# hwwang55/GraphGAN

Measured on NVIDIA H100. Metric: sampled negative edges/sec (D-sampling pass), higher is better.
Workload: dtype f32

## Files before the change

### graphgan_b200/_cabi.py

```python
import ctypes as C
import os

from . import _build

_LIB = None
ABI_VERSION = 11


class GGError(RuntimeError):
    pass


class WalkDesc(C.Structure):
    _fields_ = [
        ("n_node", C.c_int64), ("ld", C.c_int32),
        ("emb", C.c_void_p), ("bias", C.c_void_p), ("indptr", C.c_void_p), ("adj", C.c_void_p),
        ("n_roots", C.c_int64), ("roots", C.c_void_p), ("tree_bits", C.c_void_p), ("tree_words", C.c_int64),
        ("walk_ptr", C.c_void_p),
        ("n_walks", C.c_int64), ("for_d", C.c_int32), ("rng_mode", C.c_int32), ("d1_bits", C.c_void_p),
        ("seed", C.c_uint64), ("pass_tag", C.c_uint32), ("max_path", C.c_int32),
        ("stream", C.c_void_p), ("n_stream", C.c_int64), ("update_ratio", C.c_double),
        ("max_cand", C.c_int32), ("phase_mask", C.c_int32),
        ("samples", C.c_void_p), ("status", C.c_void_p), ("first_edge", C.c_void_p), ("wsteps", C.c_void_p),
        ("wsuml", C.c_void_p), ("paths", C.c_void_p), ("path_len", C.c_void_p), ("counters", C.c_void_p),
        ("scratch", C.c_void_p), ("scratch_bytes", C.c_int64), ("work_counter", C.c_void_p),
        ("edge_score", C.c_void_p), ("root_q", C.c_void_p), ("rq_ptr", C.c_void_p),
        ("hub_threshold", C.c_int32), ("no_tma", C.c_int32), ("walk_slot", C.c_void_p),
        ("s1_nq", C.c_int64), ("s1_slot", C.c_void_p), ("s1_ptr", C.c_void_p), ("s1_cnt", C.c_void_p), ("s1_n", C.c_void_p),
        ("s1_q", C.c_void_p), ("s1_ids", C.c_void_p), ("first_idx", C.c_void_p), ("s1_order", C.c_void_p), ("walk_order", C.c_void_p),
        ("flat_buf", C.c_void_p), ("flat_bytes", C.c_int64), ("flat_steps", C.c_int32), ("flat_reserved", C.c_int32),
    ]


_P, _I32, _I64, _F = C.c_void_p, C.c_int32, C.c_int64, C.c_float
SIGNATURES = {
    "gg_last_error": (C.c_char_p, []),
    "gg_abi_version": (C.c_int, []),
    "gg_hub_scores": (C.c_int, [_I64, _P, _P, _P, _P, _I32, _P, _P]),
    "gg_root_cdf": (C.c_int, [C.POINTER(WalkDesc), _P, _P, _P]),
    "gg_walk_scratch_bytes": (C.c_int, [_I32, C.POINTER(_I64)]),
    "gg_walk_flat_bytes": (C.c_int, [_I64, _I32, _I32, C.POINTER(_I64)]),
    "gg_walk_sample": (C.c_int, [C.POINTER(WalkDesc), _P]),
    "gg_generator_dist_scratch_bytes": (C.c_int, [_I64, _I64, _I64, C.POINTER(_I64)]),
    "gg_generator_dist": (C.c_int, [C.POINTER(WalkDesc), _P, _P, _P, _I64, _P]),
    "gg_game_value_scratch_bytes": (C.c_int, [_I64, _I64, C.POINTER(_I64)]),
    "gg_game_value": (C.c_int, [_I64, _I32, _P, _P, _P, _P, _I64, _P, _P, _P, _P, _P, _P, _P, _I64, _P]),
    "gg_game_value_grad_scratch_bytes": (C.c_int, [_I64, _I64, _I64, C.POINTER(_I64)]),
    "gg_game_value_grad": (C.c_int, [C.POINTER(WalkDesc), _P, _P, _P, _P, _P, _P, _P, _P, _P, _P, _I64, _P]),
    "gg_game_value_grad_d_scratch_bytes": (C.c_int, [_I64, _I32, _I64, C.POINTER(_I64)]),
    "gg_game_value_grad_d": (C.c_int, [_I64, _I32, _P, _P, _P, _P, _I64, _P, _P, _P, _P, _P, _P, _I64, _P]),
    "gg_expected_g_grad_scratch_bytes": (C.c_int, [_I64, _I64, _I64, _I32, C.POINTER(_I64)]),
    "gg_expected_g_grad": (C.c_int, [C.POINTER(WalkDesc), _P, _P, _I32, _P, _P, _P, _P, _P, _I64, _P]),
    "gg_walk_finalize": (C.c_int, [_I64, _P, _I32, _P, _P, _P, _P, _P, _P, _P, _P, _P, _P]),
    "gg_emit_d_rows": (C.c_int, [_I64, _P, _P, _P, _P, _P, _P, _P, _P, _P, _P, _P, _P]),
    "gg_bfs_scratch_bytes": (C.c_int, [_I64, _I64, C.POINTER(_I64)]),
    "gg_tree_words": (C.c_int, [_I64, C.POINTER(_I64)]),
    "gg_bfs_build": (C.c_int, [_I64, _I64, _P, _P, _I64, _P, _P, _I64, _P, _I64, _P]),
    "gg_reverse_entries": (C.c_int, [_I64, _I64, _P, _P, _P, _P, _P]),
    "gg_bfs_build_ex": (C.c_int, [_I64, _I64, _P, _P, _P, _I64, _P, _P, _I64, _P, _I64, C.c_float, C.c_int32, _P]),
    "gg_tree_parent": (C.c_int, [_I64, _P, _P, _I64, _P, _P, _I64, _P, _P]),
    "gg_pair_reward": (C.c_int, [_I64, _P, _P, _P, _P, _I32, _P, _P]),
    "gg_all_score": (C.c_int, [_I64, _P, _P, _I32, _P, _P]),
    "gg_pair_grad": (C.c_int, [_I32, _I32, _I32, _P, _P, _P, _P, _P, _I32, _F, _P, _P, _P, _P, _P, _P]),
    "gg_pair_grad_scratch_bytes": (C.c_int, [_I32, _I32, C.POINTER(_I64)]),
    "gg_pair_grad_ex": (C.c_int, [_I32, _I32, _I32, _P, _P, _P, _P, _P, _I32, _F, _P, _P, _P, _P, _P, _P, _I64, _I32, _P]),
    "gg_grad_buf_floats": (_I64, [_I32, _I32]),
    "gg_grad_merge": (C.c_int, [_I32, _I32, _I32, _P, _P, _P, _P, _P, _P, _P]),
    "gg_grad_merge_scratch_bytes": (C.c_int, [_I32, _I32, _I32, C.POINTER(_I64)]),
    "gg_grad_merge_ex": (C.c_int, [_I32, _I32, _I32, _P, _P, _P, _P, _P, _P, _P, _I64, _I32, _P]),
    "gg_comm_unique_id": (C.c_int, [_P]),
    "gg_comm_init": (C.c_int, [_P, _I32, _I32, C.POINTER(C.c_void_p)]),
    "gg_comm_destroy": (C.c_int, [_P]),
    "gg_comm_info": (C.c_int, [_P, C.POINTER(_I32), C.POINTER(_I32), C.POINTER(_I32), C.POINTER(C.c_uint64)]),
    "gg_comm_p2p_export": (C.c_int, [_P, _I64, _P]),
    "gg_comm_p2p_connect": (C.c_int, [_P, _P]),
    "gg_comm_use_p2p": (C.c_int, [_P, _I32]),
    "gg_dp_step": (C.c_int, [_P, _I32, _I32, _P, _P, _P, _I64, _I32, _P, _P, _P, _P, _P, _P, _F, _P, _P, _I32, _P, _P, _P, _P, _P,
                            _F, _F, _F, _F, _P]),
    "gg_dp_train_steps": (C.c_int, [_P, _I32, _I64, _P, _I64, _I32, _P, _P, _P, _I64, _I32, _P, _P, _P, _P, _P, _P, _F, _P, _P, _I32,
                                   _P, _P, _P, _P, _P, _F, _F, _F, _F, C.POINTER(C.c_float), C.POINTER(C.c_float), _P]),
    "gg_dp_scratch_bytes": (C.c_int, [_I32, _I32, _I32, C.POINTER(_I64)]),
    "gg_dp_step_ex": (C.c_int, [_P, _I32, _I32, _P, _P, _P, _I64, _I32, _P, _P, _P, _P, _P, _P, _F, _P, _P, _I32, _P, _P, _P, _P, _P,
                               _F, _F, _F, _F, _P, _I64, _I32, _P]),
    "gg_dp_train_steps_ex": (C.c_int, [_P, _I32, _I64, _P, _I64, _I32, _P, _P, _P, _I64, _I32, _P, _P, _P, _P, _P, _P, _F, _P, _P, _I32,
                                      _P, _P, _P, _P, _P, _F, _F, _F, _F, C.POINTER(C.c_float), C.POINTER(C.c_float), _P, _I64,
                                      _I32, _P]),
    "gg_set_adam_path": (C.c_int, [C.c_char_p]),
    "gg_adam_apply": (C.c_int, [_I64, _I32, _P, _P, _P, _P, _P, _P, _P, _P, _P, _P, _P, _F, _F, _F, _F, _P]),
    "gg_adam_apply_dense": (C.c_int, [_I64, _I32, _P, _P, _P, _P, _P, _P, _P, _P, C.c_double, _F, _F, _F, _F, _F, _F, _P]),
    "gg_train_steps": (C.c_int, [_I32, _I64, _P, _I64, _I32, _P, _P, _P, _I64, _I32, _P, _P, _P, _P, _P, _P, _F, _P, _P, _P, _P, _P,
                                _F, _F, _F, _F, C.POINTER(C.c_float), C.POINTER(C.c_float), _P]),
    "gg_train_steps_ex": (C.c_int, [_I32, _I64, _P, _I64, _I32, _P, _P, _P, _I64, _I32, _P, _P, _P, _P, _P, _P, _F, _P, _P, _P, _P, _P,
                                   _F, _F, _F, _F, C.POINTER(C.c_float), C.POINTER(C.c_float), _P, _I64, _P]),
    "gg_train_loop": (C.c_int, [_I32, _I64, _P, _I64, _I32, _P, _P, _P, _I64, _I32, _P, _P, _P, _P, _P, _P, _F, _P, _P, _P, _P, _P,
                               _F, _F, _F, _F, C.POINTER(C.c_float), C.POINTER(C.c_float), _P, _P]),
    "gg_train_fused": (C.c_int, [_I32, _I64, _P, _I64, _I32, _P, _P, _P, _I64, _I32, _P, _P, _P, _P, _P, _P, _P, _P, _F,
                                _F, _F, _F, _F, C.POINTER(C.c_float), C.POINTER(C.c_float), _P, _P]),
    "gg_pair_dot_f64": (C.c_int, [_I64, _P, _P, _P, _I32, _P, _P]),
    "gg_link_pred_acc": (C.c_int, [_I64, _P, _P, _P]),
    "gg_unpad_rows": (C.c_int, [_I64, _I32, _I32, _P, _P, _P]),
    "gg_window_pairs": (C.c_int, [_I64, _P, _P, _I32, _I32, _P, _P, _P, _P, _I64, _P]),
}


def lib():
    global _LIB
    if _LIB is None:
        path = os.environ.get("GG_LIB") or _build.LIB
        if path == _build.LIB and _build.stale():
            if os.path.exists(path) and _build.nvcc_path() is None:
                raise GGError("libgraphgan_b200.so was built from different sources and there is no nvcc to rebuild it")
            try:
                _build.build()
            except Exception as e:
                raise GGError("libgraphgan_b200.so is missing or stale and could not be built: %s" % e) from e
        try:
            handle = C.CDLL(path)
        except OSError as e:
            raise GGError("cannot load %s: %s" % (path, e)) from e
        for name, (res, args) in SIGNATURES.items():
            try:
# ... 19 lines not shown
```

### graphgan_b200/csrc/hub.cu

```cuda
#include "walk_common.cuh"

namespace gg {
namespace {

__device__ __forceinline__ float *hub_wide_row() {
    extern __shared__ __align__(16) unsigned char hub_smem[];
    return reinterpret_cast<float *>(hub_smem + (size_t)(threadIdx.x >> 5) * WIDE_ROW_BYTES);
}

__device__ __forceinline__ float *hub_group_row(int grp) {
    extern __shared__ __align__(16) unsigned char hub_smem[];
    return reinterpret_cast<float *>(hub_smem + (size_t)(4 * (threadIdx.x >> 5) + grp) * WIDE_ROW_BYTES);
}

constexpr int hub_tm_min_ctas(int cpl) { return cpl <= 2 ? 5 : cpl == 4 ? 4 : 3; }

template <int CPL>
__global__ void __launch_bounds__(WARPS_PER_CTA * 32, hub_tm_min_ctas(CPL))
hub_score_tm_kernel(long long n_items, const int4 *__restrict__ items, const int2 *__restrict__ pairs,
                    const float *__restrict__ emb, const float *__restrict__ bias, int ld, float *__restrict__ edge_score) {
    const int lane = threadIdx.x & 31, grp = lane >> 3;
    const long long warp = ((long long)blockIdx.x * blockDim.x + threadIdx.x) >> 5;
    const long long nwarps = ((long long)gridDim.x * blockDim.x) >> 5;
    for (long long t0 = 4 * warp; t0 < n_items; t0 += 4 * nwarps) {
        const int4 it = (t0 + grp < n_items) ? __ldg(items + t0 + grp) : make_int4(0, 0, 0, 0);
        const int v = it.x, n = it.z;
        const int n_warp = __reduce_max_sync(FULL, n);
        const float bv = __ldg(bias + v);
        if constexpr (CPL == WIDE_CPL) {
            float *s_row = hub_group_row(grp);
            load_row_group_wide(emb, ld, v, s_row, lane & 7);
            score_pairs_wide(emb, ld, s_row, bv, pairs + it.y, n, n_warp, edge_score, v, lane);
        } else {
            float4 c4[CPL];
            load_row<CPL>(emb, ld, v, lane & 7, c4);
            score_pairs<CPL>(emb, ld, c4, bv, pairs + it.y, n, n_warp, edge_score, v, lane);
        }
    }
}

template <int CPL>
__global__ void __launch_bounds__(WARPS_PER_CTA * 32)
root_cdf_kernel(const __grid_constant__ gg_walk_desc d, float *__restrict__ root_sc, double *__restrict__ root_q) {
    const int lane = threadIdx.x & 31;
    const long long warp = ((long long)blockIdx.x * blockDim.x + threadIdx.x) >> 5;
    const long long nwarps = ((long long)gridDim.x * blockDim.x) >> 5;
    for (long long slot = warp; slot < d.n_roots; slot += nwarps) {
        const int root = d.roots[slot];
        const long long a0 = d.indptr[root], a1 = d.indptr[root + 1], o = d.rq_ptr[slot];
        const int n = (int)(a1 - a0);
        if (n == 0) continue;
        float *sc = root_sc + o;
        if (d.edge_score && n >= d.hub_threshold) {
            for (int i = lane; i < n; i += 32) sc[i] = __ldg(d.edge_score + a0 + i);
            __syncwarp();
        } else {
            if constexpr (CPL == WIDE_CPL) {
                float *s_row = hub_wide_row();
                load_row_wide(d.emb, d.ld, root, s_row, lane);
                score_edges_wide(d.emb, d.bias, d.ld, s_row, d.adj, a0, n, sc, root, lane);
            } else {
                float4 c4[CPL];
                load_row<CPL>(d.emb, d.ld, root, lane & 7, c4);
                score_edges<CPL>(d.emb, d.bias, d.ld, c4, d.adj, a0, n, sc, root, lane);
            }
        }
        cdf_store(sc, n, root_q + o, lane);
    }
}

constexpr int hub_smem_bytes(int cpl) { return cpl == WIDE_CPL ? WARPS_PER_CTA * WIDE_ROW_BYTES : 0; }
constexpr int hub_tm_smem_bytes(int cpl) { return cpl == WIDE_CPL ? 4 * WARPS_PER_CTA * WIDE_ROW_BYTES : 0; }

}
}

extern "C" int gg_hub_scores(int64_t n_items, const int32_t *items, const int32_t *pairs, const float *emb, const float *bias,
                             int32_t ld, float *edge_score, void *stream) {
    if (n_items == 0) return 0;
    GG_REQUIRE(items && pairs && emb && bias && edge_score, "null pointer");
    GG_REQUIRE(gg::ld_supported(ld), GG_LD_MESSAGE);
    long long blocks = (n_items + 4 * gg::WARPS_PER_CTA - 1) / (4 * gg::WARPS_PER_CTA);
    const long long cap = (long long)gg::sm_count() * 8;
    if (blocks > cap) blocks = cap;
    cudaStream_t st = (cudaStream_t)stream;
    const int4 *it = reinterpret_cast<const int4 *>(items);
    const int2 *pr = reinterpret_cast<const int2 *>(pairs);
    if (ld == 512) {
        static_assert(gg::hub_tm_smem_bytes(gg::WIDE_CPL) > 48 * 1024, "the attribute is needed");
        GG_CHECK(cudaFuncSetAttribute(gg::hub_score_tm_kernel<gg::WIDE_CPL>, cudaFuncAttributeMaxDynamicSharedMemorySize,
                                      gg::hub_tm_smem_bytes(gg::WIDE_CPL)));
    }
#define GG_LAUNCH(C)                                                                                           \
    gg::hub_score_tm_kernel<C><<<(unsigned)blocks, gg::WARPS_PER_CTA * 32, gg::hub_tm_smem_bytes(C), st>>>(    \
        n_items, it, pr, emb, bias, ld, edge_score)
    switch (ld / 32) {
        case 1: GG_LAUNCH(1); break;
        case 2: GG_LAUNCH(2); break;
        case 4: GG_LAUNCH(4); break;
        case 8: GG_LAUNCH(8); break;
        case 16: GG_LAUNCH(16); break;
        default: gg::set_error("gg_hub_scores: unsupported ld %d (supported: 32, 64, 128, 256, 512)", ld); return 2;
    }
#undef GG_LAUNCH
    return gg::check_cuda(cudaGetLastError(), "hub score kernel launch");
}

extern "C" int gg_root_cdf(const gg_walk_desc *dp, float *root_sc, double *root_q, void *stream) {
    GG_REQUIRE(dp, "null descriptor");
    if (dp->n_roots == 0) return 0;
    GG_REQUIRE(root_sc && root_q, "null pointer");
    const gg_walk_desc &d = *dp;
    GG_REQUIRE(d.roots && d.indptr && d.adj && d.emb && d.bias && d.rq_ptr, "null pointer in descriptor");
    GG_REQUIRE(gg::ld_supported(d.ld), GG_LD_MESSAGE);
    if (d.n_roots == 0) return 0;
    long long blocks = (d.n_roots + gg::WARPS_PER_CTA - 1) / gg::WARPS_PER_CTA;
    const long long cap = (long long)gg::sm_count() * 8;
    if (blocks > cap) blocks = cap;
    cudaStream_t st = (cudaStream_t)stream;
    switch (d.ld / 32) {
        case 1: gg::root_cdf_kernel<1><<<(unsigned)blocks, gg::WARPS_PER_CTA * 32, 0, st>>>(d, root_sc, root_q); break;
        case 2: gg::root_cdf_kernel<2><<<(unsigned)blocks, gg::WARPS_PER_CTA * 32, 0, st>>>(d, root_sc, root_q); break;
        case 4: gg::root_cdf_kernel<4><<<(unsigned)blocks, gg::WARPS_PER_CTA * 32, 0, st>>>(d, root_sc, root_q); break;
        case 8: gg::root_cdf_kernel<8><<<(unsigned)blocks, gg::WARPS_PER_CTA * 32, 0, st>>>(d, root_sc, root_q); break;
        case 16:
            gg::root_cdf_kernel<16><<<(unsigned)blocks, gg::WARPS_PER_CTA * 32, gg::hub_smem_bytes(16), st>>>(d, root_sc, root_q);
            break;
        default: gg::set_error("gg_root_cdf: unsupported ld %d (supported: 32, 64, 128, 256, 512)", d.ld); return 2;
    }
    return gg::check_cuda(cudaGetLastError(), "root cdf kernel launch");
}
```

### graphgan_b200/graph.py

```python
import numpy as np

from . import _cabi

HUB_ITEM_CAP = 32


def read_edge_file(path):
    if path == "" or path is None:
        return np.zeros((0, 2), np.int64)
    with open(path, "r") as f:
        rows = [ln.split() for ln in f if ln.strip()]
    return np.asarray(rows, dtype=np.int64).reshape(-1, 2)


class HostGraph:

    def __init__(self, train_edges, test_edges=None, n_node=None):
        train = np.asarray(train_edges, np.int64).reshape(-1, 2)
        test = np.zeros((0, 2), np.int64) if test_edges is None else np.asarray(test_edges, np.int64).reshape(-1, 2)
        ids = np.unique(np.concatenate([train.ravel(), test.ravel()])) if (train.size + test.size) else np.zeros(0, np.int64)
        self.n_node = int(ids.shape[0]) if n_node is None else int(n_node)
        if ids.size and (ids[0] < 0 or ids[-1] >= self.n_node):
            raise ValueError("node ids must lie in [0, n_node)")
        n = self.n_node
        src = np.empty(2 * train.shape[0], np.int64)
        dst = np.empty(2 * train.shape[0], np.int64)
        src[0::2], src[1::2] = train[:, 0], train[:, 1]
        dst[0::2], dst[1::2] = train[:, 1], train[:, 0]
        order = np.argsort(src, kind="stable")
        src_s, dst_s = src[order], dst[order]
        self.raw_indptr = np.zeros(n + 1, np.int64)
        np.cumsum(np.bincount(src_s, minlength=n), out=self.raw_indptr[1:])
        self.raw_adj = dst_s.astype(np.int32)
        keep = src_s != dst_s
        s2, d2 = src_s[keep], dst_s[keep]
        key = s2 * n + d2
        _, first = np.unique(key, return_index=True)
        first.sort()
        s3, d3 = s2[first], d2[first]
        self.indptr = np.zeros(n + 1, np.int64)
        np.cumsum(np.bincount(s3, minlength=n), out=self.indptr[1:])
        self.adj = d3.astype(np.int32)
        self.max_deg = int(np.diff(self.indptr).max()) if n else 0

    @classmethod
    def from_arrays(cls, n_node, raw_indptr, raw_adj, indptr, adj):
        g = cls.__new__(cls)
        g.n_node = int(n_node)
        g.raw_indptr, g.raw_adj = np.asarray(raw_indptr, np.int64), np.asarray(raw_adj, np.int32)
        g.indptr, g.adj = np.asarray(indptr, np.int64), np.asarray(adj, np.int32)
        assert g.raw_indptr.shape == g.indptr.shape == (g.n_node + 1,)
        g.max_deg = int(np.diff(g.indptr).max()) if g.n_node else 0
        return g

    @classmethod
    def from_files(cls, train_filename, test_filename=""):
        return cls(read_edge_file(train_filename), read_edge_file(test_filename))

    def neighbors(self, i):
        return self.raw_adj[self.raw_indptr[i]:self.raw_indptr[i + 1]]

    def __getitem__(self, i):
        return self.neighbors(int(i)).tolist()

    def __len__(self):
        return self.n_node

    def degrees(self):
        return np.diff(self.raw_indptr)


class DeviceGraph:

    def __init__(self, host, device):
        import torch
        _cabi.lib()
        self.host = host
        self.device = torch.device(device)
        self.n_node = host.n_node
        self.max_deg = host.max_deg
        t = lambda a: torch.from_numpy(np.ascontiguousarray(a)).to(self.device)
        self.indptr, self.adj = t(host.indptr), t(np.concatenate([host.adj, np.zeros(4, np.int32)]))[:host.adj.shape[0]]
        same = host.raw_adj.shape == host.adj.shape and np.array_equal(host.raw_adj, host.adj)
        self.raw_indptr = self.indptr if same else t(host.raw_indptr)
        self.raw_adj = self.adj if same else t(host.raw_adj)
        self.raw_deg = t(host.degrees().astype(np.int64))
        self.n_bit_words = (host.adj.shape[0] + 31) // 32 + 1
        self.d1_bits = torch.zeros(self.n_bit_words, dtype=torch.int32, device=self.device)

    def reverse_entries(self):
        import torch
        if not hasattr(self, "_rev"):
            nnz = int(self.host.adj.shape[0])
            rev = torch.empty(max(nnz, 1), dtype=torch.int32, device=self.device)
            missing = torch.zeros(1, dtype=torch.int32, device=self.device)
            st = torch.cuda.current_stream(self.device).cuda_stream
            _cabi.check(_cabi.lib().gg_reverse_entries(self.n_node, nnz, self.indptr.data_ptr(), self.adj.data_ptr(),
                                                       rev.data_ptr(), missing.data_ptr(), st), "gg_reverse_entries")
            self._rev = rev if int(missing.item()) == 0 else None
        return self._rev

    def hub_tiles(self, threshold, item_cap=HUB_ITEM_CAP):
        import torch
        key = (int(threshold), int(item_cap))
        if getattr(self, "_hub_key", None) != key:
            dev, i64 = self.device, torch.int64
            deg_h = np.diff(self.host.indptr)
            hubs_h = np.flatnonzero(deg_h >= threshold)
            n_entries = int(deg_h[hubs_h].sum())
            items = torch.zeros((0, 4), dtype=torch.int32, device=dev)
            pairs = torch.zeros((0, 2), dtype=torch.int32, device=dev)
            if n_entries:
                hubs = torch.from_numpy(hubs_h).to(dev)
                cnt = self.indptr[hubs + 1] - self.indptr[hubs]
                src = torch.repeat_interleave(hubs, cnt, output_size=n_entries)
                run0 = torch.repeat_interleave(torch.cumsum(cnt, 0) - cnt, cnt, output_size=n_entries)
                e = self.indptr[src] + (torch.arange(n_entries, dtype=i64, device=dev) - run0)
                tgt, order = torch.sort(self.adj[e], stable=True)
                pairs = torch.stack([src[order], e[order]], 1).to(torch.int32).contiguous()
                v, run = torch.unique_consecutive(tgt, return_counts=True)
                pieces = (run + item_cap - 1) // item_cap
                n_items = int(pieces.sum().item())
                p0 = torch.cumsum(pieces, 0) - pieces
                r = torch.repeat_interleave(torch.arange(v.shape[0], dtype=i64, device=dev), pieces, output_size=n_items)
                k = torch.arange(n_items, dtype=i64, device=dev) - p0[r]
                first = (torch.cumsum(run, 0) - run)[r] + k * item_cap
                count = torch.clamp(run[r] - k * item_cap, max=item_cap)
                items = torch.stack([v[r].to(i64), first, count, torch.zeros_like(first)], 1).to(torch.int32).contiguous()
            self._hub_key = key
            self._hub = (items, pairs, int(items.shape[0]), n_entries)
            if not hasattr(self, "edge_score"):
                self.edge_score = torch.empty(self.host.adj.shape[0] + 4, dtype=torch.float32, device=self.device)[:max(self.host.adj.shape[0], 1)]
        return self._hub

    def reset_tree_mutations(self):
        self.d1_bits.zero_()
```

### graphgan_b200/sampler.py

```python
import ctypes as C
import os

import numpy as np

from . import _cabi
from ._cabi import ptr

RNG_PHILOX, RNG_STREAM = 0, 1
NOTRUN, DONE, VOID, SKIPPED = 0, 1, 2, 3
CNT = dict(steps=0, sum_l=1, accepted=2, ok_roots=3, path_overflow=4, raw_steps=5, raw_sum_l=6, stream_used=7,
           rows_gathered=8, cyc_enum=9, cyc_score=10, cyc_choose=11, cyc_step0=12, cyc_step1=13, cyc_step2p=14, cyc_walk=15)


LD_MAX = 512


def round_up(x, m):
    return (x + m - 1) // m * m


def pad_embedding(emb, device=None):
    import torch
    e = emb.float() if isinstance(emb, torch.Tensor) else torch.as_tensor(np.asarray(emb, np.float64).astype(np.float32))
    n, d = e.shape
# ... 132 lines not shown
    def __init__(self, graph, hub_threshold=128, depth1=True, hub_first=True, tma=True):
        import torch
        self.torch = torch
        self.g = graph
        self.device = graph.device
        self.lib = _cabi.lib()
        self.max_cand = graph.max_deg + 1
        self.hub_threshold = int(hub_threshold)
        self.depth1 = bool(depth1)
        self.tma = bool(tma)
        self.hub_first = bool(hub_first)
        nbytes = C.c_int64(0)
        _cabi.check(self.lib.gg_walk_scratch_bytes(self.max_cand, C.byref(nbytes)), "gg_walk_scratch_bytes")
        self.scratch = torch.empty(max(nbytes.value, 16), dtype=torch.uint8, device=self.device)
        self.work_counter = torch.zeros(1, dtype=torch.int32, device=self.device)
        self._bfs_scratch = None
        self.bfs_bottom_up_ratio = float(os.environ.get("GG_BFS_BU_RATIO", "-1"))
        self.bfs_flags = 0
        self.flat_steps = int(os.environ.get("GG_FLAT_STEPS", "4"))

    def _stream(self):
        return self.torch.cuda.current_stream(self.device).cuda_stream

    def build_trees(self, roots):
        torch = self.torch
        roots_d = roots if isinstance(roots, torch.Tensor) else torch.as_tensor(np.asarray(roots, np.int32)).to(self.device)
        R, N = int(roots_d.shape[0]), self.g.n_node
        nnz = int(self.g.adj.shape[0])
        words = C.c_int64(0)
        _cabi.check(self.lib.gg_tree_words(nnz, C.byref(words)), "gg_tree_words")
        tree_bits = torch.empty((R, words.value), dtype=torch.int32, device=self.device)
        if self._bfs_scratch is None:
            nbytes = C.c_int64(0)
            _cabi.check(self.lib.gg_bfs_scratch_bytes(N, int(self.g.adj.shape[0]), C.byref(nbytes)), "gg_bfs_scratch_bytes")
            self._bfs_scratch = torch.empty(max(nbytes.value, 16), dtype=torch.uint8, device=self.device)
        rev = self.g.reverse_entries() if self.bfs_bottom_up_ratio != 0.0 else None
        _cabi.check(self.lib.gg_bfs_build_ex(N, nnz, ptr(self.g.indptr), ptr(self.g.adj), ptr(rev) if rev is not None else None,
                                             R, ptr(roots_d), ptr(tree_bits), words.value, ptr(self._bfs_scratch),
                                             self._bfs_scratch.numel(), float(self.bfs_bottom_up_ratio), int(self.bfs_flags),
                                             self._stream()),
                    "gg_bfs_build_ex")
        return TreeBatch(roots_d, tree_bits, self.g)

    def plan(self, trees, sample_num, for_d, max_path=0):
        return WalkPlan(self, trees, sample_num, for_d, max_path)

    def _desc(self, emb, bias, plan, *, seed, pass_tag, update_ratio, rng_mode, stream, reuse, phase_mask=0):
        torch = self.torch
        assert emb.dtype == torch.float32 and emb.is_contiguous() and bias.dtype == torch.float32
        t, d = plan.trees, _cabi.WalkDesc()
        d.n_node, d.ld = self.g.n_node, int(emb.shape[1])
        d.emb, d.bias, d.indptr, d.adj = ptr(emb), ptr(bias), ptr(self.g.indptr), ptr(self.g.adj)
        d.n_roots, d.roots, d.walk_ptr, d.n_walks = plan.n_roots, ptr(t.roots), ptr(plan.walk_ptr), plan.n_walks
        d.tree_bits, d.tree_words = ptr(t.tree_bits), int(t.tree_bits.shape[1])
        d.for_d, d.rng_mode, d.d1_bits = int(plan.for_d), rng_mode, ptr(self.g.d1_bits)
        d.seed, d.pass_tag, d.max_path = seed, pass_tag, plan.max_path
        d.stream, d.n_stream = (ptr(stream), int(stream.numel())) if stream is not None else (None, 0)
        d.update_ratio, d.max_cand, d.phase_mask = float(update_ratio), self.max_cand, int(phase_mask)
        d.no_tma = 0 if self.tma else 1
        d.samples, d.status, d.first_edge, d.wsteps, d.wsuml = (ptr(plan.samples), ptr(plan.status), ptr(plan.first_edge),
                                                                 ptr(plan.wsteps), ptr(plan.wsuml))
        d.paths, d.path_len, d.counters = ptr(plan.paths), ptr(plan.path_len), ptr(plan.counters)
        d.scratch, d.scratch_bytes, d.work_counter = ptr(self.scratch), self.scratch.numel(), ptr(self.work_counter)
        d.rq_ptr, d.walk_slot = ptr(plan.rq_ptr), ptr(plan.walk_slot)
        if self.hub_first and rng_mode == RNG_PHILOX:
            d.walk_order = ptr(plan.start_order(self))
        if reuse:
            self.g.hub_tiles(self.hub_threshold)
            d.edge_score, d.hub_threshold, d.root_q = ptr(self.g.edge_score), self.hub_threshold, ptr(plan.root_q)
            if self.depth1 and rng_mode == RNG_PHILOX and plan.nq > 0 and plan.n_walks > 0:
                b = plan.depth1_buffers(self)
                d.s1_nq, d.s1_slot, d.s1_ptr, d.s1_cnt, d.s1_n = plan.nq, ptr(b["slot"]), ptr(b["ptr"]), ptr(b["cnt"]), ptr(b["n"])
                d.s1_q, d.s1_ids, d.first_idx = ptr(b["q"]), ptr(b["ids"]), ptr(b["first"])
                if self.hub_first:
                    d.s1_order = ptr(b["order"])
                if self.flat_steps > 0:
                    buf = plan.flat_buffer(self)
                    d.flat_buf, d.flat_bytes, d.flat_steps = ptr(buf), buf.numel(), self.flat_steps
        return d

    def precompute(self, emb, bias, plan, desc=None):
        d = desc if desc is not None else self._desc(emb, bias, plan, seed=0, pass_tag=0, update_ratio=1.0,
                                                     rng_mode=RNG_PHILOX, stream=None, reuse=True)
        items, pairs, n_items, _ = self.g.hub_tiles(self.hub_threshold)
        st = self._stream()
        _cabi.check(self.lib.gg_hub_scores(n_items, ptr(items), ptr(pairs), ptr(emb), ptr(bias), int(emb.shape[1]),
                                           ptr(self.g.edge_score), st), "gg_hub_scores")
        _cabi.check(self.lib.gg_root_cdf(C.byref(d), ptr(plan.root_sc), ptr(plan.root_q), st), "gg_root_cdf")

    def run(self, emb, bias, trees, sample_num, for_d, *, seed=0, pass_tag=0, update_ratio=1.0, max_path=0,
            rng_mode=RNG_PHILOX, stream=None, finalize=True, plan=None, reuse=None, precompute=True, phase_mask=0, zero_counters=True):
        if plan is None:
            plan = self.plan(trees, sample_num, for_d, max_path)
        reuse = (self.hub_threshold > 0) if reuse is None else bool(reuse)
        if zero_counters:
            plan.counters.zero_()
        d = self._desc(emb, bias, plan, seed=seed, pass_tag=pass_tag, update_ratio=update_ratio, rng_mode=rng_mode,
                       stream=stream, reuse=reuse, phase_mask=phase_mask)
        if reuse and precompute:
            self.precompute(emb, bias, plan, d)
        _cabi.check(self.lib.gg_walk_sample(C.byref(d), self._stream()), "gg_walk_sample")
        out = WalkOutput(walk_ptr=plan.walk_ptr, n_walks=plan.n_walks, n_roots=plan.n_roots, for_d=plan.for_d,
                         max_path=plan.max_path, samples=plan.samples, status=plan.status, first_edge=plan.first_edge,
                         wsteps=plan.wsteps, wsuml=plan.wsuml, paths=plan.paths, path_len=plan.path_len,
                         root_ok=plan.root_ok, counters=plan.counters, roots=trees.roots, plan=plan)
        if finalize:
            self.finalize(out)
        return out

    def distribution(self, emb, bias, trees, *, reuse=None, max_scratch_bytes=None, counters=None):
        torch = self.torch
        R, N = int(trees.roots.shape[0]), self.g.n_node
        dist = torch.empty((R, N), dtype=torch.float64, device=self.device)
        root_ok = torch.empty(R, dtype=torch.int32, device=self.device)
        for _ in self._distribution_chunks(emb, bias, trees, reuse, max_scratch_bytes, counters, dist, root_ok):
            pass
        return dist, root_ok

    def _law_desc(self, emb, bias, trees, reuse, counters):
        g = self.g
        d = _cabi.WalkDesc()
        d.n_node, d.ld = g.n_node, int(emb.shape[1])
        d.emb, d.bias, d.indptr, d.adj = ptr(emb), ptr(bias), ptr(g.indptr), ptr(g.adj)
        d.tree_words, d.d1_bits, d.counters = int(trees.tree_bits.shape[1]), ptr(g.d1_bits), ptr(counters)
        if reuse:
            items, pairs, n_items, _ = g.hub_tiles(self.hub_threshold)
            _cabi.check(self.lib.gg_hub_scores(n_items, ptr(items), ptr(pairs), ptr(emb), ptr(bias), int(emb.shape[1]),
                                               ptr(g.edge_score), self._stream()), "gg_hub_scores")
            d.edge_score, d.hub_threshold = ptr(g.edge_score), self.hub_threshold
        return d

    def _distribution_chunks(self, emb, bias, trees, reuse, max_scratch_bytes, counters, dist=None, root_ok=None,
                             extra_bytes=None):
        torch, g = self.torch, self.g
        R, N, nnz = int(trees.roots.shape[0]), g.n_node, int(g.adj.shape[0])
        if R == 0:
            return
        assert emb.dtype == torch.float32 and emb.is_contiguous() and bias.dtype == torch.float32
        reuse = (self.hub_threshold > 0) if reuse is None else bool(reuse)
        budget = int(max_scratch_bytes if max_scratch_bytes is not None else os.environ.get("GG_GDIST_SCRATCH", 2 << 30))

        def scratch_bytes(k):
            nb = C.c_int64(0)
            _cabi.check(self.lib.gg_generator_dist_scratch_bytes(N, nnz, k, C.byref(nb)), "gg_generator_dist_scratch_bytes")
            return nb.value
        per_root = scratch_bytes(1) + (extra_bytes(1) if extra_bytes is not None else 0)
        chunk = max(1, min(R, budget // max(per_root, 1), ((1 << 31) - 1) // max(N, 1)))
        scratch = torch.empty(max(scratch_bytes(chunk), 16), dtype=torch.uint8, device=self.device)
        if dist is None:
            dist = torch.empty((chunk, N), dtype=torch.float64, device=self.device)
            root_ok = torch.empty(chunk, dtype=torch.int32, device=self.device)
            rows = lambda lo, hi: (dist[:hi - lo], root_ok[:hi - lo])
        else:
            rows = lambda lo, hi: (dist[lo:hi], root_ok[lo:hi])
        d = self._law_desc(emb, bias, trees, reuse, counters)
        st = self._stream()
        for lo in range(0, R, chunk):
            hi = min(R, lo + chunk)
            dr, okr = rows(lo, hi)
            d.n_roots, d.roots, d.tree_bits = hi - lo, ptr(trees.roots[lo:hi]), ptr(trees.tree_bits[lo:hi])
            _cabi.check(self.lib.gg_generator_dist(C.byref(d), ptr(dr), ptr(okr), ptr(scratch), scratch.numel(), st),
                        "gg_generator_dist")
            yield lo, hi, dr, okr

    def game_value(self, g_emb, g_bias, d_emb, d_bias, trees, *, max_scratch_bytes=None, reuse=None):
        torch, g = self.torch, self.g
        assert d_emb.dtype == torch.float32 and d_emb.is_contiguous() and d_bias.dtype == torch.float32
        assert int(d_emb.shape[0]) == g.n_node and int(d_bias.shape[0]) == g.n_node
        R, N = int(trees.roots.shape[0]), g.n_node
        pos = torch.zeros(R, dtype=torch.float64, device=self.device)
        neg = torch.zeros(R, dtype=torch.float64, device=self.device)
        ok = torch.zeros(R, dtype=torch.int32, device=self.device)
        st, scratch = self._stream(), None
        for lo, hi, dist, root_ok in self._distribution_chunks(g_emb, g_bias, trees, reuse, max_scratch_bytes, None):
            nb = C.c_int64(0)
            _cabi.check(self.lib.gg_game_value_scratch_bytes(N, hi - lo, C.byref(nb)), "gg_game_value_scratch_bytes")
            if scratch is None or scratch.numel() < nb.value:
                scratch = torch.empty(max(nb.value, 16), dtype=torch.uint8, device=self.device)
            _cabi.check(self.lib.gg_game_value(N, int(d_emb.shape[1]), ptr(d_emb), ptr(d_bias), ptr(g.raw_indptr),
                                               ptr(g.raw_adj), hi - lo, ptr(trees.roots[lo:hi]), ptr(dist), ptr(root_ok),
                                               ptr(pos[lo:hi]), ptr(neg[lo:hi]), ptr(ok[lo:hi]), ptr(scratch),
                                               scratch.numel(), st), "gg_game_value")
        return pos, neg, ok

    def game_value_grad(self, g_emb, g_bias, d_emb, d_bias, trees, *, max_scratch_bytes=None, reuse=None):
        torch, g = self.torch, self.g
        assert g_emb.dtype == torch.float32 and g_emb.is_contiguous() and g_bias.dtype == torch.float32
        assert d_emb.dtype == torch.float32 and d_emb.is_contiguous() and d_bias.dtype == torch.float32
        assert d_emb.shape == g_emb.shape and int(d_bias.shape[0]) == g.n_node and int(g_emb.shape[0]) == g.n_node
        R, N, nnz = int(trees.roots.shape[0]), g.n_node, int(g.adj.shape[0])
        pos = torch.zeros(R, dtype=torch.float64, device=self.device)
        neg = torch.zeros(R, dtype=torch.float64, device=self.device)
        ok = torch.zeros(R, dtype=torch.int32, device=self.device)
        grad_emb = torch.zeros(tuple(g_emb.shape), dtype=torch.float64, device=self.device)
        grad_bias = torch.zeros(N, dtype=torch.float64, device=self.device)
        if R == 0:
            return pos, neg, ok, grad_emb, grad_bias
        order = torch.argsort(trees.roots.long(), stable=True)
        st_trees = trees.select(order)
        reuse = (self.hub_threshold > 0) if reuse is None else bool(reuse)
        budget = int(max_scratch_bytes if max_scratch_bytes is not None else os.environ.get("GG_GDIST_SCRATCH", 2 << 30))

        def scratch_bytes(k):
            nb = C.c_int64(0)
            _cabi.check(self.lib.gg_game_value_grad_scratch_bytes(N, nnz, k, C.byref(nb)), "gg_game_value_grad_scratch_bytes")
            return nb.value
        chunk = max(1, min(R, budget // max(scratch_bytes(1), 1), ((1 << 31) - 1) // max(N, 1)))
        scratch = torch.empty(max(scratch_bytes(chunk), 16), dtype=torch.uint8, device=self.device)
        sp, sn, so = (torch.zeros_like(x) for x in (pos, neg, ok))
        d = self._law_desc(g_emb, g_bias, st_trees, reuse, None)
        st = self._stream()
# ... 131 lines not shown
```

### include/graphgan_b200.h

```cpp
#ifndef GRAPHGAN_B200_H
#define GRAPHGAN_B200_H
#include <stdint.h>

#ifdef __cplusplus
extern "C" {
#endif

#define GG_ABI_VERSION 11

enum { GG_NOTRUN = 0, GG_DONE = 1, GG_VOID = 2, GG_SKIPPED = 3 };
enum {
    GG_RNG_PHILOX = 0,
    GG_RNG_STREAM = 1
};
enum {
    GG_CNT_STEPS = 0, GG_CNT_SUML = 1, GG_CNT_ACCEPTED = 2, GG_CNT_OK_ROOTS = 3,
    GG_CNT_PATH_OVERFLOW = 4, GG_CNT_RAW_STEPS = 5, GG_CNT_RAW_SUML = 6, GG_CNT_STREAM_USED = 7,
    GG_CNT_ROWS_GATHERED = 8,
    GG_CNT_CYC_ENUM = 9, GG_CNT_CYC_SCORE = 10, GG_CNT_CYC_CHOOSE = 11, GG_CNT_CYC_STEP0 = 12,
    GG_CNT_CYC_STEP1 = 13, GG_CNT_CYC_STEP2P = 14, GG_CNT_CYC_WALK = 15,
    GG_CNT_SLOTS = 16
};

const char *gg_last_error(void);
int gg_abi_version(void);

typedef struct gg_walk_desc {
    int64_t n_node;
    int32_t ld;
    const float *emb;
    const float *bias;
    const int64_t *indptr;
    const int32_t *adj;
    int64_t n_roots;
    const int32_t *roots;
    const uint32_t *tree_bits;
    int64_t tree_words;
    const int64_t *walk_ptr;
    int64_t n_walks;
    int32_t for_d;
    int32_t rng_mode;
    uint32_t *d1_bits;
    uint64_t seed;
    uint32_t pass_tag;
    int32_t max_path;
    const double *stream;
    int64_t n_stream;
    double update_ratio;
    int32_t max_cand;
    int32_t phase_mask;
    int32_t *samples;
    int32_t *status;
    int32_t *first_edge;
    int32_t *wsteps;
    int32_t *wsuml;
    int32_t *paths;
    int32_t *path_len;
    unsigned long long *counters;
    void *scratch;
    int64_t scratch_bytes;
    unsigned int *work_counter;
    const float *edge_score;
    const double *root_q;
    const int64_t *rq_ptr;
    int32_t hub_threshold;
    int32_t no_tma;
    const int32_t *walk_slot;
    int64_t s1_nq;
    const int32_t *s1_slot;
    const int64_t *s1_ptr;
    int32_t *s1_cnt;
    int32_t *s1_n;
    double *s1_q;
    int32_t *s1_ids;
    int32_t *first_idx;
    const int32_t *s1_order;
    const int32_t *walk_order;
    void *flat_buf;
    int64_t flat_bytes;
    int32_t flat_steps;
    int32_t flat_reserved;
} gg_walk_desc;

int gg_hub_scores(int64_t n_items, const int32_t *items, const int32_t *pairs, const float *emb, const float *bias,
                  int32_t ld, float *edge_score, void *stream);
int gg_root_cdf(const gg_walk_desc *d, float *root_sc, double *root_q, void *stream);

int gg_walk_scratch_bytes(int32_t max_cand, int64_t *bytes);
int gg_walk_flat_bytes(int64_t n_walks, int32_t hub_threshold, int32_t flat_steps, int64_t *bytes);
int gg_walk_sample(const gg_walk_desc *d, void *stream);

int gg_walk_finalize(int64_t n_roots, const int64_t *walk_ptr, int32_t for_d, int32_t *samples,
                     int32_t *status, const int32_t *first_edge, int32_t *wsteps, int32_t *wsuml,
                     int32_t *path_len, uint32_t *d1_bits, int32_t *root_ok,
                     unsigned long long *counters, void *stream);

int gg_generator_dist_scratch_bytes(int64_t n_node, int64_t nnz, int64_t n_roots, int64_t *bytes);
int gg_generator_dist(const gg_walk_desc *d, double *dist, int32_t *root_ok, void *scratch, int64_t scratch_bytes,
                      void *stream);

int gg_game_value_scratch_bytes(int64_t n_node, int64_t n_roots, int64_t *bytes);
int gg_game_value(int64_t n_node, int32_t ld, const float *emb, const float *bias, const int64_t *raw_indptr,
                  const int32_t *raw_adj, int64_t n_roots, const int32_t *roots, const double *dist,
                  const int32_t *root_ok, double *pos, double *neg, int32_t *ok, void *scratch, int64_t scratch_bytes,
                  void *stream);

int gg_game_value_grad_scratch_bytes(int64_t n_node, int64_t nnz, int64_t n_roots, int64_t *bytes);
int gg_game_value_grad(const gg_walk_desc *g, const float *d_emb, const float *d_bias, const int64_t *raw_indptr,
                       const int32_t *raw_adj, double *pos, double *neg, int32_t *ok, double *grad_emb, double *grad_bias,
                       void *scratch, int64_t scratch_bytes, void *stream);

int gg_game_value_grad_d_scratch_bytes(int64_t n_node, int32_t ld, int64_t n_roots, int64_t *bytes);
int gg_game_value_grad_d(int64_t n_node, int32_t ld, const float *emb, const float *bias, const int64_t *raw_indptr,
                         const int32_t *raw_adj, int64_t n_roots, const int32_t *roots, const double *dist,
                         const int32_t *root_ok, double *grad_emb, double *grad_bias, void *scratch, int64_t scratch_bytes,
                         void *stream);

int gg_expected_g_grad_scratch_bytes(int64_t n_node, int64_t nnz, int64_t n_roots, int32_t window, int64_t *bytes);
int gg_expected_g_grad(const gg_walk_desc *g, const float *d_emb, const float *d_bias, int32_t window, double *n_pairs,
                       int32_t *root_ok, double *grad_emb, double *grad_bias, void *scratch, int64_t scratch_bytes,
                       void *stream);

int gg_emit_d_rows(int64_t n_roots, const int32_t *roots, const int64_t *walk_ptr,
                   const int64_t *pos_indptr, const int32_t *pos_flat, const int32_t *root_ok,
                   const int32_t *samples, int64_t *row_ptr, int32_t *center, int32_t *neighbor,
                   int32_t *label, int64_t *n_rows_out, void *stream);

int gg_tree_words(int64_t nnz, int64_t *words);
int gg_bfs_scratch_bytes(int64_t n_node, int64_t nnz, int64_t *bytes);
int gg_bfs_build(int64_t n_node, int64_t nnz, const int64_t *indptr, const int32_t *adj, int64_t n_roots,
                 const int32_t *roots, uint32_t *tree_bits, int64_t tree_words, void *scratch,
                 int64_t scratch_bytes, void *stream);
#define GG_BFS_NO_SORTED_BOTTOM_UP 1
int gg_reverse_entries(int64_t n_node, int64_t nnz, const int64_t *indptr, const int32_t *adj, int32_t *rev,
                       int32_t *n_missing, void *stream);
int gg_bfs_build_ex(int64_t n_node, int64_t nnz, const int64_t *indptr, const int32_t *adj, const int32_t *rev,
                    int64_t n_roots, const int32_t *roots, uint32_t *tree_bits, int64_t tree_words, void *scratch,
                    int64_t scratch_bytes, float bottom_up_ratio, int32_t flags, void *stream);
int gg_tree_parent(int64_t n_node, const int64_t *indptr, const int32_t *adj, int64_t n_roots,
                   const int32_t *roots, const uint32_t *tree_bits, int64_t tree_words, int32_t *parent,
                   void *stream);

int gg_pair_reward(int64_t n_pairs, const int32_t *node_id, const int32_t *node_neighbor_id,
                   const float *emb, const float *bias, int32_t ld, float *reward, void *stream);
int gg_all_score(int64_t n_node, const float *emb, const float *bias, int32_t ld, float *out,
                 void *stream);

#define GG_MAX_BATCH 1024
int gg_pair_grad(int32_t mode, int32_t n_pairs, int32_t batch_total, const int32_t *node_id,
                 const int32_t *node_neighbor_id, const float *aux, const float *emb,
                 const float *bias, int32_t ld, float lambda, int32_t *n_unique, int32_t *uniq_ids,
                 float *grad_rows, float *grad_bias, int32_t *row_slot, void *stream);

#define GG_GRAD_MULTI_CTA 1
int gg_pair_grad_scratch_bytes(int32_t n_pairs, int32_t ld, int64_t *bytes);
int gg_pair_grad_ex(int32_t mode, int32_t n_pairs, int32_t batch_total, const int32_t *node_id,
                    const int32_t *node_neighbor_id, const float *aux, const float *emb, const float *bias,
                    int32_t ld, float lambda, int32_t *n_unique, int32_t *uniq_ids, float *grad_rows,
                    float *grad_bias, int32_t *row_slot, void *scratch, int64_t scratch_bytes,
                    int32_t flags, void *stream);

int64_t gg_grad_buf_floats(int32_t cap, int32_t ld);
int gg_grad_merge(int32_t world, int32_t cap, int32_t ld, const float *gathered, int32_t *n_unique,
                  int32_t *uniq_ids, float *grad_rows, float *grad_bias, int32_t *row_slot, void *stream);
int gg_grad_merge_scratch_bytes(int32_t world, int32_t cap, int32_t ld, int64_t *bytes);
int gg_grad_merge_ex(int32_t world, int32_t cap, int32_t ld, const float *gathered, int32_t *n_unique,
                     int32_t *uniq_ids, float *grad_rows, float *grad_bias, int32_t *row_slot, void *scratch,
                     int64_t scratch_bytes, int32_t flags, void *stream);
// ... 85 lines not shown
```

Before: 116.2 million.

## Score hub-hub edges once and write both directions via reverse-entry map

Builds a hub plan that splits hub-incident edges into plain pairs and hub-hub pairs. For each hub-hub edge, only the ordered direction by hub rank is kept. A new kernel computes that dot product once and writes both directed edge scores, using the reverse-entry index and each endpoint's bias. This is meant to roughly halve the dot products and embedding row gathers spent on hub-hub edges during score precompute, at the cost of extra plan-building work and a restriction to ld <= 128.

```diff
diff --git a/graphgan_b200/_cabi.py b/graphgan_b200/_cabi.py
--- a/graphgan_b200/_cabi.py
+++ b/graphgan_b200/_cabi.py
@@ -37,6 +37,7 @@
     "gg_last_error": (C.c_char_p, []),
     "gg_abi_version": (C.c_int, []),
     "gg_hub_scores": (C.c_int, [_I64, _P, _P, _P, _P, _I32, _P, _P]),
+    "gg_hub_scores_ex": (C.c_int, [_I64, _P, _P, _I64, _P, _P, _P, _P, _I32, _P, _P]),
     "gg_root_cdf": (C.c_int, [C.POINTER(WalkDesc), _P, _P, _P]),
     "gg_walk_scratch_bytes": (C.c_int, [_I32, C.POINTER(_I64)]),
     "gg_walk_flat_bytes": (C.c_int, [_I64, _I32, _I32, C.POINTER(_I64)]),
diff --git a/graphgan_b200/csrc/hub.cu b/graphgan_b200/csrc/hub.cu
--- a/graphgan_b200/csrc/hub.cu
+++ b/graphgan_b200/csrc/hub.cu
@@ -36,6 +36,63 @@
             load_row<CPL>(emb, ld, v, lane & 7, c4);
             score_pairs<CPL>(emb, ld, c4, bv, pairs + it.y, n, n_warp, edge_score, v, lane);
         }
+    }
+}
+
+template <int CPL>
+__device__ __forceinline__ void score_sym(const float *__restrict__ emb, const float *__restrict__ bias, int ld,
+                                          const float4 (&c4)[CPL], float br, const int4 *__restrict__ recs, int n, int n_warp,
+                                          float *__restrict__ out, int fallback, int lane) {
+    const int g = lane & 7;
+    const int4 fb = make_int4(fallback, 0, 0, 0);
+    int4 pa_n = (0 < n) ? __ldg(recs) : fb, pb_n = (1 < n) ? __ldg(recs + 1) : fb;
+    for (int i0 = 0; i0 < n_warp; i0 += 2) {
+        const int4 pa = pa_n, pb = pb_n;
+        pa_n = (i0 + 2 < n) ? __ldg(recs + i0 + 2) : fb;
+        pb_n = (i0 + 3 < n) ? __ldg(recs + i0 + 3) : fb;
+        float sa, sb;
+        dot2<CPL>(emb, ld, c4, pa.x, pb.x, g, sa, sb);
+        const float bwa = __ldg(bias + pa.x), bwb = __ldg(bias + pb.x);
+        if (g == 0) {
+            if (i0 < n) {
+                out[pa.y] = __fadd_rn(sa, br);
+                out[pa.z] = __fadd_rn(sa, bwa);
+            }
+            if (i0 + 1 < n) {
+                out[pb.y] = __fadd_rn(sb, br);
+                out[pb.z] = __fadd_rn(sb, bwb);
+            }
+        }
+    }
+    __syncwarp();
+}
+
+constexpr int HUB_SYM_MAX_CPL = 4;
+template <int CPL>
+__global__ void __launch_bounds__(WARPS_PER_CTA * 32, 4)
+hub_score_sym_kernel(long long n_items, const int4 *__restrict__ items, const int2 *__restrict__ pairs, long long n_sym_items,
+                     const int4 *__restrict__ sym_items, const int4 *__restrict__ sym, const float *__restrict__ emb,
+                     const float *__restrict__ bias, int ld, float *__restrict__ edge_score) {
+    const int lane = threadIdx.x & 31, grp = lane >> 3;
+    const long long warp = ((long long)blockIdx.x * blockDim.x + threadIdx.x) >> 5;
+    const long long nwarps = ((long long)gridDim.x * blockDim.x) >> 5;
+    for (long long t0 = 4 * warp; t0 < n_items; t0 += 4 * nwarps) {
+        const int4 it = (t0 + grp < n_items) ? __ldg(items + t0 + grp) : make_int4(0, 0, 0, 0);
+        const int v = it.x, n = it.z;
+        const int n_warp = __reduce_max_sync(FULL, n);
+        const float bv = __ldg(bias + v);
+        float4 c4[CPL];
+        load_row<CPL>(emb, ld, v, lane & 7, c4);
+        score_pairs<CPL>(emb, ld, c4, bv, pairs + it.y, n, n_warp, edge_score, v, lane);
+    }
+    for (long long t0 = 4 * warp; t0 < n_sym_items; t0 += 4 * nwarps) {
+        const int4 it = (t0 + grp < n_sym_items) ? __ldg(sym_items + t0 + grp) : make_int4(0, 0, 0, 0);
+        const int r = it.x, n = it.z;
+        const int n_warp = __reduce_max_sync(FULL, n);
+        const float br = __ldg(bias + r);
+        float4 c4[CPL];
+        load_row<CPL>(emb, ld, r, lane & 7, c4);
+        score_sym<CPL>(emb, bias, ld, c4, br, sym + it.y, n, n_warp, edge_score, r, lane);
     }
 }
 
@@ -106,6 +163,34 @@
     return gg::check_cuda(cudaGetLastError(), "hub score kernel launch");
 }
 
+extern "C" int gg_hub_scores_ex(int64_t n_items, const int32_t *items, const int32_t *pairs, int64_t n_sym_items,
+                                const int32_t *sym_items, const int32_t *sym, const float *emb, const float *bias, int32_t ld,
+                                float *edge_score, void *stream) {
+    GG_REQUIRE(gg::ld_supported(ld), GG_LD_MESSAGE);
+    GG_REQUIRE(n_items >= 0 && n_sym_items >= 0, "negative count");
+    if (n_sym_items == 0) return gg_hub_scores(n_items, items, pairs, emb, bias, ld, edge_score, stream);
+    GG_REQUIRE(ld / 32 <= gg::HUB_SYM_MAX_CPL, "gg_hub_scores_ex: hub-hub records need ld <= 128");
+    GG_REQUIRE((n_items == 0 || (items && pairs)) && sym_items && sym && emb && bias && edge_score, "null pointer");
+    long long blocks = (n_items + n_sym_items + 4 * gg::WARPS_PER_CTA - 1) / (4 * gg::WARPS_PER_CTA);
+    const long long cap = (long long)gg::sm_count() * 8;
+    if (blocks > cap) blocks = cap;
+    cudaStream_t st = (cudaStream_t)stream;
+    const int4 *it = reinterpret_cast<const int4 *>(items), *sit = reinterpret_cast<const int4 *>(sym_items);
+    const int2 *pr = reinterpret_cast<const int2 *>(pairs);
+    const int4 *sy = reinterpret_cast<const int4 *>(sym);
+#define GG_LAUNCH(C)                                                                                                   \
+    gg::hub_score_sym_kernel<C><<<(unsigned)blocks, gg::WARPS_PER_CTA * 32, 0, st>>>(n_items, it, pr, n_sym_items, sit, sy, \
+                                                                                      emb, bias, ld, edge_score)
+    switch (ld / 32) {
+        case 1: GG_LAUNCH(1); break;
+        case 2: GG_LAUNCH(2); break;
+        case 4: GG_LAUNCH(4); break;
+        default: gg::set_error("gg_hub_scores_ex: unsupported ld %d (supported: 32, 64, 128, 256, 512)", ld); return 2;
+    }
+#undef GG_LAUNCH
+    return gg::check_cuda(cudaGetLastError(), "hub score kernel launch");
+}
+
 extern "C" int gg_root_cdf(const gg_walk_desc *dp, float *root_sc, double *root_q, void *stream) {
     GG_REQUIRE(dp, "null descriptor");
     if (dp->n_roots == 0) return 0;
diff --git a/graphgan_b200/graph.py b/graphgan_b200/graph.py
--- a/graphgan_b200/graph.py
+++ b/graphgan_b200/graph.py
@@ -1,8 +1,27 @@
+import collections
+
 import numpy as np
 
 from . import _cabi
 
 HUB_ITEM_CAP = 32
+HUB_SYM_MAX_LD = 128
+
+
+def _cut_runs(tgt, item_cap):
+    import torch
+    dev, i64 = tgt.device, torch.int64
+    if tgt.shape[0] == 0:
+        return torch.zeros((0, 4), dtype=torch.int32, device=dev)
+    v, run = torch.unique_consecutive(tgt, return_counts=True)
+    pieces = (run + item_cap - 1) // item_cap
+    n_items = int(pieces.sum().item())
+    p0 = torch.cumsum(pieces, 0) - pieces
+    r = torch.repeat_interleave(torch.arange(v.shape[0], dtype=i64, device=dev), pieces, output_size=n_items)
+    k = torch.arange(n_items, dtype=i64, device=dev) - p0[r]
+    first = (torch.cumsum(run, 0) - run)[r] + k * item_cap
+    count = torch.clamp(run[r] - k * item_cap, max=item_cap)
+    return torch.stack([v[r].to(i64), first, count, torch.zeros_like(first)], 1).to(torch.int32).contiguous()
 
 
 def read_edge_file(path):
@@ -11,6 +30,9 @@
     with open(path, "r") as f:
         rows = [ln.split() for ln in f if ln.strip()]
     return np.asarray(rows, dtype=np.int64).reshape(-1, 2)
+
+
+HubPlan = collections.namedtuple("HubPlan", "items pairs n_items sym_items sym n_sym_items n_entries")
 
 
 class HostGraph:
@@ -118,20 +140,40 @@
                 e = self.indptr[src] + (torch.arange(n_entries, dtype=i64, device=dev) - run0)
                 tgt, order = torch.sort(self.adj[e], stable=True)
                 pairs = torch.stack([src[order], e[order]], 1).to(torch.int32).contiguous()
-                v, run = torch.unique_consecutive(tgt, return_counts=True)
-                pieces = (run + item_cap - 1) // item_cap
-                n_items = int(pieces.sum().item())
-                p0 = torch.cumsum(pieces, 0) - pieces
-                r = torch.repeat_interleave(torch.arange(v.shape[0], dtype=i64, device=dev), pieces, output_size=n_items)
-                k = torch.arange(n_items, dtype=i64, device=dev) - p0[r]
-                first = (torch.cumsum(run, 0) - run)[r] + k * item_cap
-                count = torch.clamp(run[r] - k * item_cap, max=item_cap)
-                items = torch.stack([v[r].to(i64), first, count, torch.zeros_like(first)], 1).to(torch.int32).contiguous()
+                items = _cut_runs(tgt, item_cap)
             self._hub_key = key
             self._hub = (items, pairs, int(items.shape[0]), n_entries)
             if not hasattr(self, "edge_score"):
                 self.edge_score = torch.empty(self.host.adj.shape[0] + 4, dtype=torch.float32, device=self.device)[:max(self.host.adj.shape[0], 1)]
         return self._hub
 
+    def hub_plan(self, threshold, ld, item_cap=HUB_ITEM_CAP):
+        import torch
+        key = (int(threshold), int(ld) <= HUB_SYM_MAX_LD, int(item_cap))
+        if getattr(self, "_plan_key", None) != key:
+            dev, i32, i64 = self.device, torch.int32, torch.int64
+            items, pairs, n_items, n_entries = self.hub_tiles(threshold, item_cap)
+            none = torch.zeros((0, 4), dtype=i32, device=dev)
+            plan = HubPlan(items, pairs, n_items, none, none, 0, n_entries)
+            rev = self.reverse_entries() if n_entries and ld <= HUB_SYM_MAX_LD else None
+            if rev is not None:
+                deg_h = np.diff(self.host.indptr)
+                hubs_h = np.flatnonzero(deg_h >= threshold)
+                ranked = torch.from_numpy(hubs_h[np.lexsort((hubs_h, -deg_h[hubs_h]))]).to(dev)
+                n_hubs = ranked.shape[0]
+                rank = torch.full((self.n_node,), n_hubs, dtype=i64, device=dev)
+                rank[ranked] = torch.arange(n_hubs, dtype=i64, device=dev)
+                u, e = pairs[:, 0].to(i64), pairs[:, 1].to(i64)
+                v = self.adj[e].to(i64)
+                both = rank[v] < n_hubs
+                plain, keep = ~both, both & (rank[u] < rank[v])
+                w, ewr = u[keep], e[keep]
+                sym = torch.stack([w, ewr, rev[ewr].to(i64), torch.zeros_like(w)], 1).to(i32).contiguous()
+                p_items, sym_items = _cut_runs(v[plain], item_cap), _cut_runs(v[keep], item_cap)
+                plan = HubPlan(p_items, torch.stack([u[plain], e[plain]], 1).to(i32).contiguous(), int(p_items.shape[0]),
+                               sym_items, sym, int(sym_items.shape[0]), n_entries)
+            self._plan_key, self._plan = key, plan
+        return self._plan
+
     def reset_tree_mutations(self):
         self.d1_bits.zero_()
diff --git a/graphgan_b200/sampler.py b/graphgan_b200/sampler.py
--- a/graphgan_b200/sampler.py
+++ b/graphgan_b200/sampler.py
@@ -238,11 +238,15 @@
     def precompute(self, emb, bias, plan, desc=None):
         d = desc if desc is not None else self._desc(emb, bias, plan, seed=0, pass_tag=0, update_ratio=1.0,
                                                      rng_mode=RNG_PHILOX, stream=None, reuse=True)
-        items, pairs, n_items, _ = self.g.hub_tiles(self.hub_threshold)
-        st = self._stream()
-        _cabi.check(self.lib.gg_hub_scores(n_items, ptr(items), ptr(pairs), ptr(emb), ptr(bias), int(emb.shape[1]),
-                                           ptr(self.g.edge_score), st), "gg_hub_scores")
-        _cabi.check(self.lib.gg_root_cdf(C.byref(d), ptr(plan.root_sc), ptr(plan.root_q), st), "gg_root_cdf")
+        self._hub_scores(emb, bias)
+        _cabi.check(self.lib.gg_root_cdf(C.byref(d), ptr(plan.root_sc), ptr(plan.root_q), self._stream()), "gg_root_cdf")
+
+    def _hub_scores(self, emb, bias):
+        ld = int(emb.shape[1])
+        p = self.g.hub_plan(self.hub_threshold, ld)
+        _cabi.check(self.lib.gg_hub_scores_ex(p.n_items, ptr(p.items), ptr(p.pairs), p.n_sym_items, ptr(p.sym_items),
+                                              ptr(p.sym), ptr(emb), ptr(bias), ld, ptr(self.g.edge_score), self._stream()),
+                    "gg_hub_scores_ex")
 
     def run(self, emb, bias, trees, sample_num, for_d, *, seed=0, pass_tag=0, update_ratio=1.0, max_path=0,
             rng_mode=RNG_PHILOX, stream=None, finalize=True, plan=None, reuse=None, precompute=True, phase_mask=0, zero_counters=True):
@@ -280,9 +284,7 @@
         d.emb, d.bias, d.indptr, d.adj = ptr(emb), ptr(bias), ptr(g.indptr), ptr(g.adj)
         d.tree_words, d.d1_bits, d.counters = int(trees.tree_bits.shape[1]), ptr(g.d1_bits), ptr(counters)
         if reuse:
-            items, pairs, n_items, _ = g.hub_tiles(self.hub_threshold)
-            _cabi.check(self.lib.gg_hub_scores(n_items, ptr(items), ptr(pairs), ptr(emb), ptr(bias), int(emb.shape[1]),
-                                               ptr(g.edge_score), self._stream()), "gg_hub_scores")
+            self._hub_scores(emb, bias)
             d.edge_score, d.hub_threshold = ptr(g.edge_score), self.hub_threshold
         return d
 
diff --git a/include/graphgan_b200.h b/include/graphgan_b200.h
--- a/include/graphgan_b200.h
+++ b/include/graphgan_b200.h
@@ -84,6 +84,8 @@
 
 int gg_hub_scores(int64_t n_items, const int32_t *items, const int32_t *pairs, const float *emb, const float *bias,
                   int32_t ld, float *edge_score, void *stream);
+int gg_hub_scores_ex(int64_t n_items, const int32_t *items, const int32_t *pairs, int64_t n_sym_items, const int32_t *sym_items,
+                     const int32_t *sym, const float *emb, const float *bias, int32_t ld, float *edge_score, void *stream);
 int gg_root_cdf(const gg_walk_desc *d, float *root_sc, double *root_q, void *stream);
 
 int gg_walk_scratch_bytes(int32_t max_cand, int64_t *bytes);
```

Result: no change. 116.2 million, median of 6 (+0.0%).
